# ntampellini/TSCoDe

Measured on AMD Instinct MI355X. Metric: conformers/sec, 100k x 50-atom prune_conformers pipeline (embed -> clash mask -> RMSD prune), higher is better.
Workload: dtype f64

## Files before the change

tscode_amd/csrc/local_pass.hpp:

```cpp
#pragma once
#include "rmsd.hpp"
#include "sieve.hpp"

namespace tsc {

constexpr int LP_MAX_ROWS = 2048;
constexpr int LP_WAVES = 4;
constexpr int LP_THREADS = LP_WAVES * 64;
constexpr int LP_TI = 16;
#ifndef TSC_LP_TPB
#define TSC_LP_TPB 4
#endif
constexpr int LP_TILES_PER_BLOCK = TSC_LP_TPB;
constexpr int LP_QCAP = LP_TI * 64 + 64;
constexpr int LP_WORDS = LP_MAX_ROWS / 64;
constexpr int LP_TICKET_GROUPS = 16;
#ifndef TSC_LP_OCC
#define TSC_LP_OCC 4
#endif
constexpr int LP_OCCUPANCY = TSC_LP_OCC;

struct LocalPassArgs {
    int h;
    int use_cache;
    int nb_regular;
    int nb_last;
    int c_lo;
    int n_reg;
    unsigned long long *exch;
    double thr, maxdev_thr, half_h_thr2, two_thr2, desc_limit;
    const unsigned *dmax_bits;
    unsigned long long *dbg;
};

struct LocalTickets {
    unsigned group[LP_TICKET_GROUPS][32];
    unsigned top;
    unsigned pad[31];
};

#ifdef TSC_DBG_STAMPS
#define LP_STAGE_IN(exact)                                \
    do {                                                  \
        if (!n_stages) TSC_STAMP(2);                      \
        n_stages += (exact) ? 65536 : 1;                  \
    } while (0)
#define LP_STAGE_OUT() TSC_STAMP(4)
#define LP_STAGE_COUNT()                                                                                                             \
    do {                                                                                                                             \
        if (a.dbg && (threadIdx.x & 63) == 0) a.dbg[size_t(blockIdx.x) * 32 + (threadIdx.x >> 6) * 8 + 6] = (unsigned long long)n_stages; \
    } while (0)
#else
#define LP_STAGE_IN(exact) do { } while (0)
#define LP_STAGE_OUT() do { } while (0)
#define LP_STAGE_COUNT() do { } while (0)
#endif

__device__ inline unsigned long long lds_extract64(const unsigned long long *bits, int start) {
    const int w = start >> 6, sh = start & 63;
    const unsigned long long lo = bits[w] >> sh;
    const unsigned long long hi = sh ? (bits[w + 1] << (64 - sh)) : 0ull;
    return lo | hi;
}

// ... 5 lines not shown
    unsigned long long my_sb = 0ull;
    for (int j = cv.first; j < cv.count; ++j) {
        const ViewPass vp = cv.pass[j];
        bool ok = false;
        if (removed) {
            const int c = int(((unsigned long long)unsigned(a) * vp.magic) >> vp.shift);
            if (c * vp.cs == a && c < vp.k) ok = b < ((c == vp.k - 1) ? cv.n : vp.cs * (c + 1));
        }
        unsigned long long left = __ballot(ok);
        if (!left) continue;
        unsigned long long *v = cv.views + int64_t(j) * cv.stride;
        if (ok) atomicOr(&v[b >> 6], 1ull << (b & 63));
        for (bool primary = true; left; primary = false) {
            const int leader = __ffsll((long long)left) - 1;
            const int word = __shfl(b >> 16, leader);
            const bool same = ok && (b >> 16) == word;
            unsigned long long sb = same ? 1ull << ((b >> 10) & 63) : 0ull;
            for (int off = 32; off > 0; off >>= 1) sb |= __shfl_xor(sb, off);
            if (primary) {
                if (lane == j - cv.first) my_word = int64_t(j) * cv.stride + cv.bit_words + word, my_sb = sb;
            } else if (lane == leader) {
                unsigned long long *ds = v + cv.bit_words + word;
                if ((__hip_atomic_load(ds, __ATOMIC_RELAXED, __HIP_MEMORY_SCOPE_AGENT) & sb) != sb) atomicOr(ds, sb);
            }
            left &= ~__ballot(same);
        }
    }
    if (my_sb) {
        unsigned long long *ds = cv.views + my_word;
        if ((__hip_atomic_load(ds, __ATOMIC_RELAXED, __HIP_MEMORY_SCOPE_AGENT) & my_sb) != my_sb) atomicOr(ds, my_sb);
    }
}

inline __global__ __launch_bounds__(LP_THREADS, LP_OCCUPANCY) void k_pass_chunks(PassGeom g, LocalPassArgs a, PruneState *__restrict__ st, uint8_t *__restrict__ mask,
                                                             unsigned long long *__restrict__ bits, int bit_words,
                                                             const unsigned long long *__restrict__ dbit, const double *__restrict__ heavy,
                                                             const double *__restrict__ Gall, const float *__restrict__ D,
                                                             CacheViews cv, PassCounters *__restrict__ cnt, int32_t *__restrict__ bsum, int block_items,
                                                             StepCtx sc, StepArgs next, LocalTickets *__restrict__ tickets, DeriveArgs dv) {
    __shared__ unsigned long long s_mb[LP_WORDS + 2], s_db[LP_WORDS + 2];
    __shared__ unsigned short s_wpre[LP_WORDS + 2];
    __shared__ unsigned short s_act[LP_MAX_ROWS], s_cend[LP_MAX_ROWS];
    __shared__ int s_best[LP_MAX_ROWS];
    __shared__ unsigned short s_queue[LP_WAVES][LP_QCAP], s_exq[LP_WAVES][128];
    __shared__ __attribute__((aligned(16))) float s_rowdesc[LP_WAVES][LP_TI * DW];
    __shared__ double s_jacobi[LP_WAVES][32];
    __shared__ unsigned long long s_stat[8];
    __shared__ int s_A, s_anydb, s_last, s_open[2];
    static_assert(DW == 16 && LP_TI * DW == 256, "row staging: 4 rows x 16 components per 64 lanes");

    const int tid = threadIdx.x, lane = tid & 63;
    const int wid = __builtin_amdgcn_readfirstlane(tid >> 6);
    TSC_STAMP(0);
    int c, j, nb;
    {
        const int reg_blocks = a.n_reg * a.nb_regular;
        if (int(blockIdx.x) < reg_blocks) {
            c = int(blockIdx.x) / a.nb_regular, j = int(blockIdx.x) - c * a.nb_regular, nb = a.nb_regular;
            c += a.c_lo;
        } else {
            c = g.k - 1, j = int(blockIdx.x) - reg_blocks, nb = a.nb_last;
        }
    }
    const int first = c * g.cs;
    const int L = ((c == g.k - 1) ? g.n : first + g.cs) - first;
    const int nw = (L + 63) >> 6;
// ... 54 lines not shown
        }
        __syncthreads();
        const int A = __builtin_amdgcn_readfirstlane(s_A);
        auto rank_of = [&](int t) { return int(s_wpre[t >> 6]) + __popcll(s_mb[t >> 6] & ((t & 63) ? (~0ull >> (64 - (t & 63))) : 0ull)); };
        for (int t = tid; t < L; t += LP_THREADS)
            if ((s_mb[t >> 6] >> (t & 63)) & 1ull) s_act[rank_of(t)] = (unsigned short)t;
        __syncthreads();
        const int n_tiles = (A + LP_TI - 1) / LP_TI;
        const int my_tiles = n_tiles > j ? (n_tiles - j + nb - 1) / nb : 0;
        for (int idx = tid; idx < my_tiles * LP_TI; idx += LP_THREADS) {
            const int r = (j + (idx / LP_TI) * nb) * LP_TI + (idx % LP_TI);
            if (r >= A) continue;
            const int t = s_act[r];
            int found = L;
            if (s_anydb) {
                const int len = L - t - 1;
                for (int d0 = 1; d0 <= len; d0 += 64) {
                    unsigned long long w = lds_extract64(s_mb, t + d0) & lds_extract64(s_db, d0);
                    const int rem = len - d0 + 1;
                    if (rem < 64) w &= (1ull << rem) - 1ull;
                    if (w) {
                        found = t + d0 + __ffsll((long long)w) - 1;
                        break;
                    }
                }
            }
            s_cend[r] = (unsigned short)(found >= L ? A : rank_of(found));
            s_best[r] = INT_MAX;
        }
        __syncthreads();
        TSC_STAMP(1);

        const int h3 = a.h * 3;
        const float limit32 = screen_limit32(__uint_as_float(dmax_raw), a.desc_limit);
        auto place_in = [](unsigned long long m) __attribute__((always_inline)) {
            return int(__builtin_amdgcn_mbcnt_hi(unsigned(m >> 32), __builtin_amdgcn_mbcnt_lo(unsigned(m), 0u)));
        };
        unsigned short *queue = s_queue[wid], *exq = s_exq[wid];
        float *rowdesc = s_rowdesc[wid];
        double *jac = s_jacobi[wid];
        int tile_no = 0;
        for (int rt = j; rt < n_tiles; rt += nb, ++tile_no) {
            if ((tile_no % LP_WAVES) != wid) continue;
            const int r0 = rt * LP_TI;
            const int nrows = min(LP_TI, A - r0);
            const int my_cend = lane < nrows ? int(s_cend[r0 + lane]) : 0;
            const bool live0 = lane < nrows && my_cend > r0 + lane + 1;
            unsigned alive = unsigned(__builtin_amdgcn_ballot_w64(live0));
            if (!alive) continue;
            int cmax = live0 ? my_cend : 0;
#pragma unroll
            for (int off = 32; off > 0; off >>= 1) cmax = max(cmax, __shfl_xor(cmax, off));
            cmax = __builtin_amdgcn_readfirstlane(cmax);
            float row_part[4];
#pragma unroll
            for (int q = 0; q < 4; ++q) {
                const int rr = min(r0 + 4 * q + (lane >> 4), A - 1);
                row_part[q] = D[int64_t(first + s_act[rr]) * DW + (lane & 15)];
            }
            int qn = 0, qe = 0;

            auto note_similar = [&](bool sim, int t, int col) __attribute__((always_inline)) {
                if (sim) atomicMin(&s_best[r0 + t], col);
                unsigned long long sm = __builtin_amdgcn_ballot_w64(sim);
                while (sm) {
                    const int l = __ffsll((long long)sm) - 1;
                    sm &= sm - 1;
                    alive &= ~(1u << __builtin_amdgcn_readlane(t, l));
                }
            };
            auto exact_stage = [&](int base, int cnt) __attribute__((always_inline)) {
                LP_STAGE_IN(true);
                int lpp = 64;
                while (lpp > 1 && 64 / lpp < cnt) lpp >>= 1;
                const int grp = lane / lpp, sub = lane - grp * lpp;
                bool sim = false, degenerate = false;
                int t = 0, col = 0;
                unsigned ent = 0;
                if (grp < cnt) {
                    ent = exq[base + grp];
                    t = int(ent >> 12), col = int(ent & 0xfffu);
                    const int i = first + s_act[r0 + t], jj = first + s_act[col];
                    const double *pp = heavy + int64_t(i) * h3, *pq = heavy + int64_t(jj) * h3;
                    const double Gi = Gall[i], Gj = Gall[jj];
                    double H[9], e[4];
                    pair_H(pp, pq, a.h, sub, lpp, H);
                    if (rotation_quaternion_fast(H, Gi, Gj, e)) {
                        const unsigned ent2 = reinterpret_cast<const volatile unsigned short *>(exq)[base + grp];
                        t = int(ent2 >> 12), col = int(ent2 & 0xfffu);
                        const int i2 = first + s_act[r0 + t], j2 = first + s_act[col];
                        double rm, md;
// ... 38 lines not shown
                int t = 0, col = 0;
                if (grp < cnt) {
                    e = queue[base + grp];
                    t = int(e >> 12), col = int(e & 0xfffu);
                    const int i = first + s_act[r0 + t], jj = first + s_act[col];
                    const double half_sum = 0.5 * (Gall[i] + Gall[jj]);
                    double H[9];
                    pair_H(heavy + int64_t(i) * h3, heavy + int64_t(jj) * h3, a.h, sub, lpp, H);
                    const int verdict = pair_verdict(H, half_sum, a.half_h_thr2, a.two_thr2, a.h);
                    cand = sub == 0 && verdict == PAIR_UNDECIDED;
                    sim = sub == 0 && verdict == PAIR_SIMILAR;
                }
                note_similar(sim, t, col);
                const unsigned long long m = __builtin_amdgcn_ballot_w64(cand);
                if (m) {
                    if (cand) exq[qe + place_in(m)] = (unsigned short)e;
                    qe += __popcll(m);
                }
                n_eval = __builtin_amdgcn_readfirstlane(n_eval + cnt);
                n_exact = __builtin_amdgcn_readfirstlane(n_exact + __popcll(m));
                __builtin_amdgcn_wave_barrier();
                LP_STAGE_OUT();
            };

            auto load_cols = [&](int c0, f32x2 (&dst)[KD]) __attribute__((always_inline)) {
                const f32x4 *src = reinterpret_cast<const f32x4 *>(D + int64_t(first + s_act[min(c0 + lane, A - 1)]) * DW);
#pragma unroll
                for (int k = 0; k < KD / 2; ++k) {
                    const f32x4 v = src[k];
                    dst[2 * k] = f32x2{v.x, v.y};
                    dst[2 * k + 1] = f32x2{v.z, v.w};
                }
            };
            f32x2 dq[KD], dq_next[KD];
            int c0 = (r0 + 1) & ~63;
            load_cols(c0, dq_next);
#pragma unroll
            for (int q = 0; q < 4; ++q) rowdesc[64 * q + lane] = row_part[q];
            __builtin_amdgcn_wave_barrier();
            for (bool screening = true;;) {
                if (screening) {
                    const int col = c0 + lane;
#pragma unroll
                    for (int k = 0; k < KD; ++k) dq[k] = dq_next[k];
                    if (c0 + 64 < cmax) load_cols(c0 + 64, dq_next);
                    const bool here = lane < nrows && ((alive >> lane) & 1u) && my_cend > c0 && r0 + lane < c0 + 63;
                    unsigned rows = unsigned(__builtin_amdgcn_ballot_w64(here));
                    my_screened += here ? max(0, min(my_cend, c0 + 64) - max(r0 + lane + 1, c0)) : 0;
                    while (rows) {
                        const int t = __ffs(rows) - 1;
                        rows &= rows - 1;
                        const int r = r0 + t;
                        const int ce = __builtin_amdgcn_readlane(my_cend, t);
                        const f32x2 *dr = reinterpret_cast<const f32x2 *>(rowdesc + t * DW);
                        f32x2 s2 = {0.0f, 0.0f};
#pragma unroll
                        for (int k = 0; k < KD; ++k) {
                            const f32x2 d = dr[k] - dq[k];
                            s2 = __builtin_elementwise_fma(d, d, s2);
                        }
                        const bool pass = col > r && col < ce && !(fmaxf(s2.x, s2.y) > limit32);
                        const unsigned long long m = __builtin_amdgcn_ballot_w64(pass);
                        if (m) {
                            if (pass) queue[qn + place_in(m)] = (unsigned short)((unsigned(t) << 12) | unsigned(col));
                            qn += __popcll(m);
                        }
                    }
                    c0 += 64;
                    __builtin_amdgcn_wave_barrier();
                }
                auto pending = [&]() __attribute__((always_inline)) { return qe >= 64 || qn >= 64 || (!screening && (qn | qe) != 0); };
                if (pending()) {
                    do {
                        if (qe >= 64 || qn == 0) {
                            const int cnt = min(qe, 64);
                            exact_stage(qe - cnt, cnt);
                            qe -= cnt;
                        } else {
                            const int cnt = min(qn, 64);
                            sign_stage(qn - cnt, cnt);
                            qn -= cnt;
                        }
                    } while (pending());
                    if (!screening) break;
                    load_cols(c0, dq_next);
                } else if (!screening) {
                    break;
                }
                screening = c0 < cmax && alive;
            }
        }
        for (int off = 8; off > 0; off >>= 1) my_screened += __shfl_xor(my_screened, off);
        const unsigned long long n_screened = (unsigned long long)my_screened;
        TSC_STAMP(3);
        __syncthreads();

        unsigned long long n_evaluated = 0, n_removed = 0;
        for (int rt = j; rt < n_tiles; rt += nb) {
            const int r = rt * LP_TI + lane;
            if (((rt - j) / nb) % LP_WAVES != wid) continue;
            bool removed = false;
            int my_block = -1, delta = 0;
            unsigned long long ev = 0;
            if (lane < LP_TI && r < A) {
                const int b = s_best[r];
                if (b != INT_MAX) {
                    const int t_r = s_act[r], t_b = s_act[b];
                    if (a.exch) {
                        atomicOr(&a.exch[(first + t_r) >> 6], 1ull << ((first + t_r) & 63));
                    } else {
                        mask[first + t_r] = 0;
                        atomicAnd(&mbit_next[(first + t_r) >> 6], ~(1ull << ((first + t_r) & 63)));
                        my_block = (first + t_r) / block_items;
                    }
                    delta = t_b - t_r;
                    removed = true;
                    ev = (unsigned long long)(b - r);
                } else {
                    ev = (unsigned long long)(int(s_cend[r]) - r - 1);
                }
            }
// ... 51 lines not shown
```

tscode_amd/csrc/pairs_sorted.hip:

```cpp
#include "prune_host.hpp"

int launch_rmsd_sieve_sorted(bool f32, hipStream_t st, dim3 grid, hipEvent_t e0, hipEvent_t e1, const double *heavy, const int32_t *act, const double *Gall,
                             const int32_t *cend, int32_t *best, PassCounters *counters, const PruneState *state, const SieveArgs &a, const CullArgs &ca,
                             int my_tiles, int n_seg) {
    if (f32) hipExtLaunchKernelGGL(k_rmsd_sieve_sorted<true>, grid, dim3(256), 0, st, e0, e1, 0, heavy, act, Gall, cend, best, counters, state, a, ca, my_tiles, n_seg);
    else hipExtLaunchKernelGGL(k_rmsd_sieve_sorted<false>, grid, dim3(256), 0, st, e0, e1, 0, heavy, act, Gall, cend, best, counters, state, a, ca, my_tiles, n_seg);
    TSC_HIP(hipGetLastError());
    return 0;
}

int launch_pass_chunks(hipStream_t st, unsigned blocks, hipEvent_t e0, hipEvent_t e1, const PassGeom &g, const LocalPassArgs &a, PruneState *state, uint8_t *mask,
                       unsigned long long *bits, int bit_words, const unsigned long long *view, const double *heavy, const double *Gall, const float *Dall,
                       const CacheViews &cv, PassCounters *counters, int32_t *bsum, int block_items, const StepCtx &sc, const StepArgs &sa, LocalTickets *tickets,
                       const DeriveArgs &dv) {
    hipExtLaunchKernelGGL(k_pass_chunks, dim3(blocks), dim3(LP_THREADS), 0, st, e0, e1, 0, g, a, state, mask, bits, bit_words, view, heavy, Gall, Dall, cv, counters,
                          bsum, block_items, sc, sa, tickets, dv);
    TSC_HIP(hipGetLastError());
    return 0;
}
```

tscode_amd/csrc/prune.hip:

```cpp
#include "call.hpp"
#include "prune_host.hpp"


extern "C" __attribute__((visibility("default"))) int tsc_rmsd_pairs_dev(tsc_ctx *c, const double *heavy, int64_t n_structs, int h, const int32_t *pairs, int64_t n_pairs,
                                  double *rmsd, double *maxdev) {
    TSC_API_GUARD_BEGIN
    TSC_REQUIRE(c && heavy && pairs && rmsd && maxdev, "tsc_rmsd_pairs_dev: null argument");
    TSC_REQUIRE(n_structs >= 0 && h > 0 && n_pairs >= 0, "bad sizes");
    if (n_pairs == 0) return 0;
    DeviceGuard guard(c->device);
    hipLaunchKernelGGL(k_rmsd_pairs, dim3(grid_for(n_pairs, 256)), dim3(256), 0, c->stream, heavy, h, pairs, n_pairs, rmsd, maxdev);
    TSC_HIP(hipGetLastError());
    return 0;
    TSC_API_GUARD_END
}

extern "C" __attribute__((visibility("default"))) int tsc_rmsd_pairs(tsc_ctx *c, const double *heavy, int64_t n_structs, int h, const int32_t *pairs, int64_t n_pairs,
                              double *rmsd, double *maxdev) {
    TSC_API_GUARD_BEGIN
    TSC_REQUIRE(c && heavy && pairs && rmsd && maxdev, "tsc_rmsd_pairs: null argument");
    TSC_REQUIRE(n_structs >= 0 && h > 0 && n_pairs >= 0, "bad sizes");
    for (int64_t k = 0; k < 2 * n_pairs; ++k)
        TSC_REQUIRE(pairs[k] >= 0 && pairs[k] < n_structs, "pairs[%lld] = %d out of range", (long long)k, pairs[k]);
    if (n_pairs == 0) return 0;
// ... 189 lines not shown
        p->mask = mask_buffer;
    else if (!rc)
        rc = palloc(p, size_t(n), &p->mask);
    if (!rc) rc = palloc(p, size_t(n), &p->act);
    if (!rc) rc = palloc(p, size_t(n), &p->cend);
    if (!rc) rc = palloc(p, size_t(n), &p->best);
    if (!rc) rc = palloc(p, size_t(p->n_blocks) + 1, &p->bsum);
    if (!rc) rc = palloc(p, size_t(p->n_blocks) + 1, &p->boff);
    if (!rc) rc = palloc(p, size_t(n) / 16 + 8, &p->tile_cmax);
    if (!rc) rc = palloc(p, size_t(n) / 16 + 8, &p->tile_done);
    if (!rc) rc = palloc(p, 2 * p->bit_words, &p->bits);
    p->dsum_words = p->bit_words / 1024 + 4;
    p->n_views = 0;
    for (int slot = 0; slot < TSC_MAX_PASSES; ++slot) p->view_of_slot[slot] = (pass_can_run(n, slot) && mode == 0) ? p->n_views++ : -1;
    if (!rc) rc = palloc(p, std::max<size_t>(1, size_t(p->n_views) * (p->bit_words + p->dsum_words)), &p->views);
    if (!rc) rc = palloc(p, TSC_MAX_PASSES, &p->view_pass);
    if (!rc) rc = palloc(p, TSC_MAX_PASSES, &p->counters_all);
    if (!rc) rc = palloc(p, TSC_MAX_PASSES, &p->state_all);
    p->counters = p->counters_all, p->state = p->state_all;
    if (!rc) rc = palloc(p, TSC_MAX_PASSES, &p->records);
    const bool own_desc = !(ext && ext->D);
    if (!rc && p->algo == ALGO_SIEVE) {
        if (own_desc) {
            rc = palloc(p, size_t(n) * DW, &p->Dall);
            if (!rc) rc = palloc(p, size_t(n), &p->Gall);
            if (!rc) rc = palloc(p, 4, &p->dmax_bits);
        } else {
            p->Dall = ext->D, p->Gall = ext->G, p->dmax_bits = ext->dmax_bits;
        }
        if (!rc) rc = palloc(p, size_t(n) * DW, &p->Dc);
        p->mm64 = c->opt.sieve_mm == 2 || (c->opt.sieve_mm == 1 && n >= c->opt.mm_min_n);
        const bool want_mm = p->mm64 || c->opt.sieve_mm16 != 0;
        if (!rc && want_mm) rc = palloc(p, size_t(n) * MM_REC_HALVES, &p->Dh);
        if (!rc && want_heavy32(c->opt, double(n) * h * 24.0)) {
            if (ext && ext->heavy32) {
                p->heavy32 = ext->heavy32;
            } else {
                rc = palloc(p, size_t(n) * heavy32_pitch(h), &p->heavy32);
                if (!rc) hipLaunchKernelGGL(k_heavy32, dim3(unsigned(std::min<int64_t>(ceil_div<int64_t>(n * heavy32_pitch(h), 256), 65536))), dim3(256), 0, c->stream,
                                            heavy_dev, n, h, p->heavy32);
            }
        }
    }
    if (!rc) rc = palloc(p, 1, &p->tickets);
    if (!rc && p->algo == ALGO_TILE) {
        const size_t hp3 = size_t(p->hp) * 3;
        rc = palloc(p, size_t(p->npad) * hp3, &p->Xr);
        if (!rc) rc = palloc(p, size_t(p->npad) * hp3, &p->Xc);
        if (!rc) rc = palloc(p, size_t(p->npad), &p->G);
    }
    if (!rc) {
        hipStream_t st = c->stream;
        int first_slot = -1;
        for (int slot = 0; slot < TSC_MAX_PASSES && first_slot < 0; ++slot)
            if (pass_can_run(n, slot)) first_slot = slot;
        p->opened_slot = first_slot;
        InitArgs ia;
        memset(&ia, 0, sizeof(ia));
        ia.n = n, ia.mask = p->mask, ia.bits = p->bits, ia.bit_words = int(p->bit_words);
        ia.views = p->views, ia.view_words = int64_t(p->n_views) * int64_t(p->bit_words + p->dsum_words), ia.view_pass = p->view_pass, ia.n_views = p->n_views;
        for (int slot = 0; slot < TSC_MAX_PASSES; ++slot)
            if (p->view_of_slot[slot] >= 0) ia.sched[p->view_of_slot[slot]] = view_pass(int(n), int(KS[slot]));
        ia.st = p->state_all, ia.rec = p->records, ia.n_rec = TSC_MAX_PASSES, ia.cnt = p->counters_all;
        ia.bsum = p->bsum, ia.boff = p->boff, ia.n_blocks = p->n_blocks, ia.block_items = SCAN_TILE;
        ia.dmax_bits = own_desc ? p->dmax_bits : nullptr;
        ia.zero_words = reinterpret_cast<unsigned *>(p->tickets), ia.n_zero_words = int64_t(sizeof(*p->tickets) / sizeof(unsigned));
        ia.act = p->act, ia.first_slot = first_slot, ia.first_k = first_slot >= 0 ? (long long)KS[first_slot] : 0ll, ia.first_algo = p->algo;
        ia.tile_done = p->tile_done, ia.n_tile_done = n / 16 + 8;
        hipLaunchKernelGGL(k_init_run, dim3(grid_for(n / 8 + 1, 256, 512)), dim3(256), 0, st, ia);
        hipError_t e = hipGetLastError();
        if (e == hipSuccess && p->Xc) e = hipMemsetAsync(p->Xc, 0, size_t(p->npad) * p->hp * 3 * sizeof(double), st);
        if (e == hipSuccess && p->Xr) e = hipMemsetAsync(p->Xr, 0, size_t(p->npad) * p->hp * 3 * sizeof(double), st);
        if (e == hipSuccess && p->G) e = hipMemsetAsync(p->G, 0, size_t(p->npad) * sizeof(double), st);
        if (e != hipSuccess) rc = fail(TSC_ERR_HIP, "prune state setup failed: %s", hipGetErrorString(e));
    }
    if (!rc && p->Dall && own_desc) rc = build_descriptors(p, basis);
    if (rc) {
        tsc_prune_destroy(p);
        return rc;
    }
    *out = p;
    return 0;
}


extern "C" __attribute__((visibility("default"))) int tsc_prune_create(tsc_ctx *c, const double *heavy_dev, int64_t n, int h, double rmsd_thr, int mode, tsc_prune **out) {
    TSC_API_GUARD_BEGIN
    TSC_REQUIRE(c != nullptr, "tsc_prune_create: null argument");
    if (c->xd_valid && c->xd_h == h && c->xd_heavy == heavy_dev && n <= c->xd_cap && c->opt.prune_algo != ALGO_TILE) {
        ExternalDescriptors ext;
        ext.D = c->xd_D, ext.G = c->xd_G, ext.dmax_bits = c->xd_dmax;
        ext.heavy32 = c->xd_h32_valid ? c->xd_heavy32 : nullptr;
        c->xd_valid = false;
        TSC_TRY(prune_create_impl(c, heavy_dev, n, h, rmsd_thr, mode, nullptr, out, nullptr, &ext));
        std::lock_guard<std::mutex> lock(c->runs_mutex);
        (*out)->borrows_xd = true;
        ++c->xd_borrowers;
        return 0;
    }
    c->xd_valid = false;
    const double *basis = pending_basis(c, h);
    if (basis) {
        DeviceGuard guard(c->device);
        TSC_HIP(hipStreamWaitEvent(c->stream, c->ev_join, 0));
    }
    c->eb_valid = false;
    return prune_create_impl(c, heavy_dev, n, h, rmsd_thr, mode, nullptr, out, basis);
    TSC_API_GUARD_END
}
// ... 103 lines not shown
        fa.tile_done = p->tile_done, fa.tickets = p->cur_range ? &p->tickets->pass : nullptr, fa.n_tiles = unsigned(w.n_tiles);
        fa.sc = step_ctx(p, p->cur_range);
        int nxt = -1;
        fa.next = next_step_args(p, &nxt);
        if (!p->cur_range) p->last_local = false;
    }
    const bool trim = c->opt.sieve_cpl == 2 && c->opt.sieve_trim;
    if (form.mm16) {
        TSC_TRY(launch_rmsd_sieve_mm16(p->cur_fused, a.heavy32 != nullptr, w.mm16_waves, st, w.grid, ev.e0, ev.e1, p->heavy, (const int32_t *)p->act,
                                       (const double *)p->Gall, (const _Float16 *)p->Dh, (const int32_t *)p->cend, p->best, p->counters,
                                       (const PruneState *)p->state, a, fa));
        return 0;
    }
    if (form.mm) {
        TSC_TRY(launch_rmsd_sieve_mm(p->cur_fused, a.heavy32 != nullptr, st, w.grid, ev.e0, ev.e1, p->heavy, (const int32_t *)p->act, (const double *)p->Gall,
                                     (const float *)p->Dc, (const _Float16 *)p->Dh, (const int32_t *)p->cend, p->best, p->counters, (const PruneState *)p->state, a,
                                     fa));
        return 0;
    }
    TSC_TRY((p->cur_fused ? launch_rmsd_sieve_fused : launch_rmsd_sieve_plain)(
        c->opt.sieve_cpl, trim, trim && a.heavy32 != nullptr, st, w.grid, ev.e0, ev.e1, p->heavy, (const int32_t *)p->act, (const double *)p->Gall, (const float *)p->Dc,
        (const int32_t *)p->cend, p->best, p->counters, (const PruneState *)p->state, a, fa));
    TSC_HIP(hipGetLastError());
    return 0;
}

static int local_pass(tsc_prune *p, const PassGeom &g, const PassRows &r, bool range) {
    const LocalPlan l = plan_local(p->n, p->cur_k, r);
    LocalPassArgs a;
    a.h = p->h, a.use_cache = (p->mode == 0);
    a.nb_regular = l.nb_regular, a.nb_last = l.nb_last;
    a.c_lo = int(r.c_lo), a.n_reg = l.n_reg;
    a.exch = range ? p->exch : nullptr;
    a.dbg = nullptr;
#ifdef TSC_DBG_STAMPS
    if (p->ctx->opt.dbg_stamp_k == p->cur_k) TSC_TRY(stamp_buffer(p->ctx, int64_t(l.blocks) * 4, &a.dbg));
#endif
    put_screen_thresholds(p, a);
    int nxt = -1;
    const StepArgs sa = next_step_args(p, &nxt);
    const PairEvents ev = pair_events(p, 2);
    TSC_TRY(launch_pass_chunks(p->ctx->stream, unsigned(l.blocks), ev.e0, ev.e1, g, a, p->state, p->mask, p->bits, int(p->bit_words), view_of_open_pass(p), p->heavy,
                               (const double *)p->Gall, (const float *)p->Dall, later_views(p), p->counters, p->bsum, SCAN_TILE, step_ctx(p, range), sa,
                               range ? &p->tickets->local : nullptr, derive_args(p)));
    if (!range) p->last_local = true;
    return 0;
}

static int open_rows(tsc_prune *p, const PassGeom &g, const PassShape &s, bool range) {
    tsc_ctx *c = p->ctx;
    hipStream_t st = c->stream;
    const OpenPlan o = plan_open_rows(s.rows_ub);
    OpenArgs oa;
    oa.use_cache = (p->mode == 0), oa.fused = (s.fused && range) ? 1 : 0, oa.lds_cap = std::min(c->opt.open_lds_blocks, OPEN_LDS_BLOCKS);
    oa.view = view_of_open_pass(p), oa.bits = p->bits, oa.bit_words = int(p->bit_words);
    oa.boff = p->boff, oa.n_blocks = p->n_blocks, oa.block_items = SCAN_TILE;
    oa.n_tiles = o.n_tiles, oa.tickets = &p->tickets->pass;
    oa.dv = derive_args(p), oa.bsum = p->bsum, oa.boff_out = p->boff;
    oa.rank_of = s.culled ? p->rank_of : nullptr;
    oa.Dh = p->Dh, oa.dmax_bits = p->dmax_bits;
    oa.dbg = nullptr;
#ifdef TSC_DBG_STAMPS
    if (c->opt.dbg_stamp_k == -p->cur_k) TSC_TRY(stamp_buffer(c, int64_t(o.stamp_blocks) * 4, &oa.dbg));
#endif
    int nxt = -1;
    const StepArgs sa = s.fused ? next_step_args(p, &nxt) : StepArgs{-1, -1, 0ll, 0, -1};
    static_assert(SCAN_TILE == 64 * SCAN_BLOCK_WORDS && DW == DESC_WORDS, "k_open_rows");
    hipLaunchKernelGGL(k_open_rows, dim3(o.blocks), dim3(256), 0, st, g, oa, step_ctx(p, range), sa, p->act, p->cend, p->best, p->tile_cmax, (const float *)p->Dall,
                       s.need_dc ? p->Dc : nullptr);
    if (p->algo == ALGO_TILE) {
        const int hp3 = p->hp * 3;
        size_t lds = size_t(64) * (hp3 + 1) * sizeof(double);
        hipLaunchKernelGGL(k_compact_coords, dim3(ceil_div(s.rows_ub, 64)), dim3(256), lds, st, p->heavy, p->h, hp3, p->act, (const PruneState *)p->state, p->Xr,
                           p->Xc, p->npad, p->G);
    }
// ... 561 lines not shown
```

tscode_amd/csrc/prune_host.hpp:

```cpp
#pragma once

#include "pass_plan.hpp"
#include "scan.hpp"


static const double KS[TSC_MAX_PASSES] = {5e5, 2e5, 1e5, 5e4, 2e4, 1e4, 5000, 2000, 1000, 500, 200, 100, 50, 20, 10, 5, 2, 1};

static_assert(MAX_SLOTS == TSC_MAX_PASSES, "one cache view per schedule slot");

static inline bool pass_can_run(int64_t n, int slot) {
    const int64_t k = int64_t(KS[slot]);
    return k == 1 || 20 * k < n;
}

struct tsc_prune {
    tsc_ctx *ctx = nullptr;
    const double *heavy = nullptr;
    int64_t n = 0, npad = 0;
    int h = 0, hp = 0;
    double thr = 0;
    int mode = 0;
    int algo = ALGO_SIEVE;
    uint8_t *mask = nullptr;
    int32_t *act = nullptr, *cend = nullptr, *best = nullptr;
    int32_t *bsum = nullptr, *boff = nullptr, *tile_cmax = nullptr, *tile_done = nullptr;
    int n_blocks = 0;
    unsigned long long *bits = nullptr;
    unsigned long long *views = nullptr;
    ViewPass *view_pass = nullptr;
    int view_of_slot[TSC_MAX_PASSES];
    int n_views = 0;
    size_t bit_words = 0, dsum_words = 0;
    bool cur_fused = false;
    double *Xr = nullptr, *Xc = nullptr, *G = nullptr;
    float *Dall = nullptr;
    float *Dc = nullptr;
    bool mm64 = false;
    _Float16 *Dh = nullptr;
    double *Gall = nullptr;
    struct Tickets {
        PassTickets pass;
        LocalTickets local;
    } *tickets = nullptr;
    bool cur_local = false;
    int32_t *morton_order = nullptr, *rank_of = nullptr, *crank = nullptr, *cbase = nullptr, *cfill = nullptr, *blk_cnt = nullptr;
    float *Ds = nullptr, *cbox = nullptr, *rbox = nullptr;
    int32_t *cstruct = nullptr;
    _Float16 *Dhs = nullptr;
    float *heavy32 = nullptr;
    bool morton_sorted = false;
    int part_rank = 0, part_world = 1, part_min_chunks = 0;
    unsigned long long *exch = nullptr;
    bool cur_range = false;
    int range_ready_slot = -1;
    bool views_split = false;
    uint8_t *export_mask_host = nullptr;
    unsigned *dmax_bits = nullptr;
    PassCounters *counters_all = nullptr;
    PruneState *state_all = nullptr;
    PassCounters *counters = nullptr;
    PruneState *state = nullptr;
    PassRecord *records = nullptr;
    std::vector<void *> blocks;
    int next_ks = 0;
    int cur_slot = -1;
    int last_slot = -1;
    int opened_slot = -1;
    bool derive_prev = false;
    int derive_slot = -1;
    bool last_local = false, derive_local = false;
    int64_t cur_k = 0;
// ... 65 lines not shown
static inline const unsigned long long *view_of_open_pass(const tsc_prune *p) {
    return p->mode == 0 ? p->views + size_t(p->view_of_slot[p->cur_slot]) * (p->bit_words + p->dsum_words) : p->views;
}

static inline ApplyArgs apply_args(const tsc_prune *p) {
    ApplyArgs a;
    a.g = PassGeom{int(p->n), int(p->cur_k), int(p->n / p->cur_k)};
    a.act = p->act, a.cend = p->cend, a.best = p->best, a.mask = p->mask, a.bits = p->bits, a.bit_words = int(p->bit_words);
    a.bsum = p->bsum, a.block_items = SCAN_TILE, a.cv = later_views(p);
    a.exch = p->cur_range ? p->exch : nullptr;
    return a;
}

int launch_rmsd_tile(int hp, hipStream_t st, dim3 grid, hipEvent_t e0, hipEvent_t e1, const double *Xr, const double *Xc, const double *G, const int32_t *cend,
                     int32_t *best, PassCounters *counters, const PruneState *state, const TileArgs &a);
int launch_rmsd_sieve_fused(int cpl, bool trim, bool f32, hipStream_t st, dim3 grid, hipEvent_t e0, hipEvent_t e1, const double *heavy, const int32_t *act,
                            const double *Gall, const float *Dc, const int32_t *cend, int32_t *best, PassCounters *counters, const PruneState *state,
                            const SieveArgs &a, const FusedApply &fa);
int launch_rmsd_sieve_plain(int cpl, bool trim, bool f32, hipStream_t st, dim3 grid, hipEvent_t e0, hipEvent_t e1, const double *heavy, const int32_t *act,
                            const double *Gall, const float *Dc, const int32_t *cend, int32_t *best, PassCounters *counters, const PruneState *state,
                            const SieveArgs &a, const FusedApply &fa);
int launch_rmsd_sieve_mm(bool fused, bool f32, hipStream_t st, dim3 grid, hipEvent_t e0, hipEvent_t e1, const double *heavy, const int32_t *act, const double *Gall,
                         const float *Dc, const _Float16 *Dh, const int32_t *cend, int32_t *best, PassCounters *counters, const PruneState *state, const SieveArgs &a,
                         const FusedApply &fa);
int launch_rmsd_sieve_sorted(bool f32, hipStream_t st, dim3 grid, hipEvent_t e0, hipEvent_t e1, const double *heavy, const int32_t *act, const double *Gall,
                             const int32_t *cend, int32_t *best, PassCounters *counters, const PruneState *state, const SieveArgs &a, const CullArgs &ca,
                             int my_tiles, int n_seg);
int launch_rmsd_sieve_mm16(bool fused, bool f32, int waves, hipStream_t st, dim3 grid, hipEvent_t e0, hipEvent_t e1, const double *heavy, const int32_t *act, const double *Gall,
                           const _Float16 *Dh, const int32_t *cend, int32_t *best, PassCounters *counters, const PruneState *state,
                           const SieveArgs &a, const FusedApply &fa);
int launch_rmsd_sieve_sorted_mm(bool f32, hipStream_t st, dim3 grid, hipEvent_t e0, hipEvent_t e1, const double *heavy, const int32_t *act, const double *Gall,
                                const int32_t *cend, int32_t *best, PassCounters *counters, const PruneState *state, const SieveArgs &a, const CullArgs &ca,
                                const CullMmArgs &cm, int n_groups, int n_seg);
int launch_pass_chunks(hipStream_t st, unsigned blocks, hipEvent_t e0, hipEvent_t e1, const PassGeom &g, const LocalPassArgs &a, PruneState *state, uint8_t *mask,
                       unsigned long long *bits, int bit_words, const unsigned long long *view, const double *heavy, const double *Gall, const float *Dall,
                       const CacheViews &cv, PassCounters *counters, int32_t *bsum, int block_items, const StepCtx &sc, const StepArgs &sa, LocalTickets *tickets,
                       const DeriveArgs &dv);
```

tscode_amd/csrc/rmsd.hpp:

```cpp
#pragma once
#include "common.hpp"
#include "mm_record.hpp"
#include "scan.hpp"

namespace tsc {


__device__ inline void top_eigvec4(double A[4][4], double q[4]) {
    double V[4][4];
#pragma unroll
    for (int i = 0; i < 4; ++i)
#pragma unroll
        for (int j = 0; j < 4; ++j) V[i][j] = (i == j) ? 1.0 : 0.0;
    for (int sweep = 0; sweep < 16; ++sweep) {
        double off = 0.0, dia = 0.0;
#pragma unroll
        for (int i = 0; i < 4; ++i) {
            dia += A[i][i] * A[i][i];
#pragma unroll
            for (int j = i + 1; j < 4; ++j) off += A[i][j] * A[i][j];
        }
        if (!(off > 1e-30 * dia)) break;
#pragma unroll
        for (int p = 0; p < 3; ++p) {
// ... 301 lines not shown
                unsigned long long *ds = v + cv.bit_words + word;
                if ((__hip_atomic_load(ds, __ATOMIC_RELAXED, __HIP_MEMORY_SCOPE_AGENT) & sb) != sb) atomicOr(ds, sb);
            }
            left &= ~__ballot(same);
        }
    }
}

struct InitArgs {
    int64_t n;
    uint8_t *mask;
    unsigned long long *bits;
    int bit_words;
    unsigned long long *views;
    int64_t view_words;
    ViewPass *view_pass;
    int n_views;
    ViewPass sched[MAX_SLOTS];
    PruneState *st;
    PassRecord *rec;
    int n_rec;
    PassCounters *cnt;
    int32_t *bsum, *boff;
    int n_blocks, block_items;
    unsigned *dmax_bits;
    unsigned *zero_words;
    int64_t n_zero_words;
    int32_t *tile_done;
    int64_t n_tile_done;
    int32_t *act;
    int first_slot;
    long long first_k;
    int first_algo;
};
inline __global__ __launch_bounds__(256) void k_init_run(InitArgs a) {
    const int64_t n = a.n;
    const int64_t tid = int64_t(blockIdx.x) * blockDim.x + threadIdx.x, stride = int64_t(gridDim.x) * blockDim.x;
    unsigned long long *m8 = reinterpret_cast<unsigned long long *>(a.mask);
    for (int64_t e = tid; e < n / 8; e += stride) m8[e] = 0x0101010101010101ull;
    for (int64_t e = (n / 8) * 8 + tid; e < n; e += stride) a.mask[e] = 1;
    for (int64_t e = tid; e < n; e += stride) a.act[e] = int32_t(e);
    for (int64_t e = tid; e < a.bit_words; e += stride) {
        const int64_t lo = e * 64;
        const unsigned long long w = lo + 64 <= n ? ~0ull : (lo >= n ? 0ull : ((1ull << (n - lo)) - 1ull));
        a.bits[e] = w, a.bits[a.bit_words + e] = w;
    }
    for (int64_t e = tid; e < a.view_words; e += stride) a.views[e] = 0;
    unsigned long long *c = &a.cnt->w[0][0];
    for (int64_t e = tid; e < int64_t(MAX_SLOTS) * CNT_BUCKETS * CNT_WORDS; e += stride) c[e] = 0;
    for (int64_t e = tid; e < a.n_zero_words; e += stride) a.zero_words[e] = 0;
    for (int64_t e = tid; e < a.n_tile_done; e += stride) a.tile_done[e] = 0;
    char *r = reinterpret_cast<char *>(a.rec);
    for (int64_t e = tid; e < int64_t(a.n_rec) * int64_t(sizeof(PassRecord)); e += stride)
        if (int(e / int64_t(sizeof(PassRecord))) != a.first_slot) r[e] = 0;
    for (int64_t e = tid; e <= a.n_blocks; e += stride) {
        const int64_t lo = e * a.block_items;
        if (e < a.n_blocks) a.bsum[e] = int32_t(lo >= n ? 0 : (n - lo < a.block_items ? n - lo : a.block_items));
        a.boff[e] = int32_t(lo >= n ? n : lo);
    }
    if (tid < a.n_views) a.view_pass[tid] = a.sched[tid];
    if (tid == 0) {
        if (a.dmax_bits) *a.dmax_bits = 0;
        for (int s = 0; s < MAX_SLOTS; ++s) {
            PruneState *ss = a.st + s;
            ss->n_active = int(n), ss->pass_on = 0, ss->A = int(n), ss->ticket = 0, ss->bitsel = 0, ss->row_lo = 0, ss->cull_on = 0;
        }
        PruneState *st = a.st + (a.first_slot >= 0 ? a.first_slot : 0);
        if (a.first_slot >= 0) {
            const int on = (a.first_k == 1 || 20 * a.first_k < (long long)n) ? 1 : 0;
            PassRecord &fr = a.rec[a.first_slot];
            fr.k = a.first_k, fr.n_before = fr.n_after = (long long)n, fr.on = on, fr.algo = a.first_algo;
            fr.formed = fr.exact = fr.screened = fr.evaluated = fr.removed = 0;
            st->pass_on = on;
        }
// ... 957 lines not shown
```

Measured before the change: 152.0 million.

## Screen chunk-local pass pairs with f16 MFMA descriptor records

Adds an MFMA-based screening path to the chunk-local pass kernel, templated on MM. It builds f16 descriptor records, either in the init kernel or in a separate kernel, and computes 16x16 similarity blocks with mfma_f32_16x16x16f16. Threshold hits are extracted via sign bits and pushed into the exact-stage queue. This replaces the scalar f32 per-lane descriptor screen. It costs extra memory for the records plus a record-building pass, and relies on the conservativeness of the f16 screening bound.

```diff
diff --git a/tscode_amd/csrc/local_pass.hpp b/tscode_amd/csrc/local_pass.hpp
--- a/tscode_amd/csrc/local_pass.hpp
+++ b/tscode_amd/csrc/local_pass.hpp
@@ -1,6 +1,7 @@
 #pragma once
 #include "rmsd.hpp"
 #include "sieve.hpp"
+#include "mm.hpp"
 
 namespace tsc {
 
@@ -30,6 +31,7 @@
     unsigned long long *exch;
     double thr, maxdev_thr, half_h_thr2, two_thr2, desc_limit;
     const unsigned *dmax_bits;
+    const _Float16 *rec;
     unsigned long long *dbg;
 };
 
@@ -101,6 +103,9 @@
     }
 }
 
+constexpr int LP_MM_BLOCKS = 64 / MM_STEP;
+
+template <bool MM>
 inline __global__ __launch_bounds__(LP_THREADS, LP_OCCUPANCY) void k_pass_chunks(PassGeom g, LocalPassArgs a, PruneState *__restrict__ st, uint8_t *__restrict__ mask,
                                                              unsigned long long *__restrict__ bits, int bit_words,
                                                              const unsigned long long *__restrict__ dbit, const double *__restrict__ heavy,
@@ -221,7 +226,9 @@
         TSC_STAMP(1);
 
         const int h3 = a.h * 3;
-        const float limit32 = screen_limit32(__uint_as_float(dmax_raw), a.desc_limit);
+        [[maybe_unused]] const float limit32 = MM ? 0.0f : screen_limit32(__uint_as_float(dmax_raw), a.desc_limit);
+        [[maybe_unused]] const float limit_mm = MM ? __uint_as_float(__builtin_amdgcn_readfirstlane(__float_as_uint(screen_limit_mm(dmax_raw, a.desc_limit)))) : 0.0f;
+        [[maybe_unused]] const int g4 = lane >> 4, rc = lane & 15;
         auto place_in = [](unsigned long long m) __attribute__((always_inline)) {
             return int(__builtin_amdgcn_mbcnt_hi(unsigned(m >> 32), __builtin_amdgcn_mbcnt_lo(unsigned(m), 0u)));
         };
@@ -241,11 +248,18 @@
 #pragma unroll
             for (int off = 32; off > 0; off >>= 1) cmax = max(cmax, __shfl_xor(cmax, off));
             cmax = __builtin_amdgcn_readfirstlane(cmax);
-            float row_part[4];
-#pragma unroll
-            for (int q = 0; q < 4; ++q) {
-                const int rr = min(r0 + 4 * q + (lane >> 4), A - 1);
-                row_part[q] = D[int64_t(first + s_act[rr]) * DW + (lane & 15)];
+            [[maybe_unused]] float row_part[4];
+            [[maybe_unused]] f16x4 Ar[NFAM];
+            if constexpr (MM) {
+                const _Float16 *rr = a.rec + int64_t(first + s_act[min(r0 + rc, A - 1)]) * MM_REC_HALVES;
+#pragma unroll
+                for (int fam = 0; fam < NFAM; ++fam) Ar[fam] = mm_load_A(rr, fam, g4);
+            } else {
+#pragma unroll
+                for (int q = 0; q < 4; ++q) {
+                    const int rr = min(r0 + 4 * q + (lane >> 4), A - 1);
+                    row_part[q] = D[int64_t(first + s_act[rr]) * DW + (lane & 15)];
+                }
             }
             int qn = 0, qe = 0;
 
@@ -350,14 +364,73 @@
                     dst[2 * k + 1] = f32x2{v.z, v.w};
                 }
             };
-            f32x2 dq[KD], dq_next[KD];
+            auto load_recs = [&](int c0, f16x4 (&dst)[LP_MM_BLOCKS][NFAM]) __attribute__((always_inline)) {
+#pragma unroll
+                for (int b = 0; b < LP_MM_BLOCKS; ++b)
+                    mm_load_B2(a.rec + int64_t(first + s_act[min(c0 + MM_STEP * b + rc, A - 1)]) * MM_REC_HALVES, g4, dst[b]);
+            };
+            static_assert(NFAM == 2 && LP_TI * DW == 64 * 4, "a lane's two operands are the 16 bytes at its place in the row area");
+            auto put_rows = [&]() __attribute__((always_inline)) {
+                const f32x2 lo = __builtin_bit_cast(f32x2, Ar[0]), hi = __builtin_bit_cast(f32x2, Ar[1]);
+                *reinterpret_cast<f32x4 *>(rowdesc + 4 * lane) = f32x4{lo.x, lo.y, hi.x, hi.y};
+            };
+            auto get_rows = [&]() __attribute__((always_inline)) {
+                const f32x4 v = *reinterpret_cast<const f32x4 *>(rowdesc + 4 * lane);
+                const f32x2 lo = {v.x, v.y}, hi = {v.z, v.w};
+                Ar[0] = __builtin_bit_cast(f16x4, lo), Ar[1] = __builtin_bit_cast(f16x4, hi);
+                if (g4 == 2 && !((alive >> rc) & 1u)) Ar[0][0] = _Float16(__builtin_inff());
+            };
+            [[maybe_unused]] f32x2 dq[KD], dq_next[KD];
+            [[maybe_unused]] f16x4 Bq[LP_MM_BLOCKS][NFAM];
             int c0 = (r0 + 1) & ~63;
-            load_cols(c0, dq_next);
-#pragma unroll
-            for (int q = 0; q < 4; ++q) rowdesc[64 * q + lane] = row_part[q];
+            if constexpr (MM) {
+                put_rows();
+            } else {
+                load_cols(c0, dq_next);
+#pragma unroll
+                for (int q = 0; q < 4; ++q) rowdesc[64 * q + lane] = row_part[q];
+            }
             __builtin_amdgcn_wave_barrier();
             for (bool screening = true;;) {
-                if (screening) {
+                if constexpr (MM) {
+                    if (screening) {
+                        load_recs(c0, Bq);
+                        const bool here = lane < nrows && ((alive >> lane) & 1u) && my_cend > c0 && r0 + lane < c0 + 63;
+                        my_screened += here ? max(0, min(my_cend, c0 + 64) - max(r0 + lane + 1, c0)) : 0;
+                        get_rows();
+                        unsigned m0 = 0, m1 = 0;
+#pragma unroll
+                        for (int b = 0; b < LP_MM_BLOCKS; ++b) {
+                            const f32x4 z = {-limit_mm, -limit_mm, -limit_mm, -limit_mm};
+                            const f32x4 s0 = __builtin_amdgcn_mfma_f32_16x16x16f16(Ar[0], Bq[b][0], z, 0, 0, 0);
+                            const f32x4 s1 = __builtin_amdgcn_mfma_f32_16x16x16f16(Ar[1], Bq[b][1], z, 0, 0, 0);
+#pragma unroll
+                            for (int i = 0; i < 4; ++i) {
+                                m0 = __builtin_amdgcn_alignbit(m0, __float_as_uint(s0[i]), 31);
+                                m1 = __builtin_amdgcn_alignbit(m1, __float_as_uint(s1[i]), 31);
+                            }
+                        }
+                        static_assert(4 * LP_MM_BLOCKS == 16, "16 values per lane and family: moved to the top half for the count of leading zeros");
+                        unsigned hits = (m0 & m1) << 16;
+                        while (__builtin_amdgcn_ballot_w64(hits != 0u)) {
+                            bool keep = false;
+                            unsigned ent = 0;
+                            if (hits) {
+                                const int jv = __builtin_clz(hits);
+                                hits &= ~(0x80000000u >> jv);
+                                const int row = 4 * g4 + (jv & 3), col = c0 + MM_STEP * (jv >> 2) + rc;
+                                keep = col > r0 + row && ((alive >> row) & 1u) && col < int(s_cend[r0 + row]);
+                                ent = (unsigned(row) << 12) | unsigned(col);
+                            }
+                            const unsigned long long km = __builtin_amdgcn_ballot_w64(keep);
+                            if (keep) queue[qn + place_in(km)] = (unsigned short)ent;
+                            qn += __popcll(km);
+                        }
+                        c0 += 64;
+                        alive &= ~unsigned(__builtin_amdgcn_ballot_w64(lane < nrows && ((alive >> lane) & 1u) && my_cend <= c0));
+                        __builtin_amdgcn_wave_barrier();
+                    }
+                } else if (screening) {
                     const int col = c0 + lane;
 #pragma unroll
                     for (int k = 0; k < KD; ++k) dq[k] = dq_next[k];
@@ -399,12 +472,14 @@
                             sign_stage(qn - cnt, cnt);
                             qn -= cnt;
                         }
+                        if constexpr (MM) alive = unsigned(__builtin_amdgcn_readfirstlane(int(alive)));
                     } while (pending());
                     if (!screening) break;
-                    load_cols(c0, dq_next);
+                    if constexpr (!MM) load_cols(c0, dq_next);
                 } else if (!screening) {
                     break;
                 }
+                if constexpr (MM) alive = unsigned(__builtin_amdgcn_readfirstlane(int(alive)));
                 screening = c0 < cmax && alive;
             }
         }
diff --git a/tscode_amd/csrc/pairs_sorted.hip b/tscode_amd/csrc/pairs_sorted.hip
--- a/tscode_amd/csrc/pairs_sorted.hip
+++ b/tscode_amd/csrc/pairs_sorted.hip
@@ -9,12 +9,14 @@
     return 0;
 }
 
-int launch_pass_chunks(hipStream_t st, unsigned blocks, hipEvent_t e0, hipEvent_t e1, const PassGeom &g, const LocalPassArgs &a, PruneState *state, uint8_t *mask,
+int launch_pass_chunks(bool mm, hipStream_t st, unsigned blocks, hipEvent_t e0, hipEvent_t e1, const PassGeom &g, const LocalPassArgs &a, PruneState *state, uint8_t *mask,
                        unsigned long long *bits, int bit_words, const unsigned long long *view, const double *heavy, const double *Gall, const float *Dall,
                        const CacheViews &cv, PassCounters *counters, int32_t *bsum, int block_items, const StepCtx &sc, const StepArgs &sa, LocalTickets *tickets,
                        const DeriveArgs &dv) {
-    hipExtLaunchKernelGGL(k_pass_chunks, dim3(blocks), dim3(LP_THREADS), 0, st, e0, e1, 0, g, a, state, mask, bits, bit_words, view, heavy, Gall, Dall, cv, counters,
-                          bsum, block_items, sc, sa, tickets, dv);
+    if (mm) hipExtLaunchKernelGGL(k_pass_chunks<true>, dim3(blocks), dim3(LP_THREADS), 0, st, e0, e1, 0, g, a, state, mask, bits, bit_words, view, heavy, Gall, Dall, cv,
+                                  counters, bsum, block_items, sc, sa, tickets, dv);
+    else hipExtLaunchKernelGGL(k_pass_chunks<false>, dim3(blocks), dim3(LP_THREADS), 0, st, e0, e1, 0, g, a, state, mask, bits, bit_words, view, heavy, Gall, Dall, cv,
+                               counters, bsum, block_items, sc, sa, tickets, dv);
     TSC_HIP(hipGetLastError());
     return 0;
 }
diff --git a/tscode_amd/csrc/prune.hip b/tscode_amd/csrc/prune.hip
--- a/tscode_amd/csrc/prune.hip
+++ b/tscode_amd/csrc/prune.hip
@@ -245,6 +245,10 @@
         p->mm64 = c->opt.sieve_mm == 2 || (c->opt.sieve_mm == 1 && n >= c->opt.mm_min_n);
         const bool want_mm = p->mm64 || c->opt.sieve_mm16 != 0;
         if (!rc && want_mm) rc = palloc(p, size_t(n) * MM_REC_HALVES, &p->Dh);
+        bool local_possible = false;
+        for (int slot = 0; slot < TSC_MAX_PASSES; ++slot)
+            local_possible = local_possible || (pass_can_run(n, slot) && n / int64_t(KS[slot]) <= std::min(LP_MAX_ROWS, c->opt.local_max_chunk));
+        if (!rc && c->opt.sieve_mm16 != 0 && c->opt.local_pass != 0 && local_possible) rc = palloc(p, size_t(n) * MM_REC_HALVES, &p->Drec);
         if (!rc && want_heavy32(c->opt, double(n) * h * 24.0)) {
             if (ext && ext->heavy32) {
                 p->heavy32 = ext->heavy32;
@@ -280,7 +284,9 @@
         ia.zero_words = reinterpret_cast<unsigned *>(p->tickets), ia.n_zero_words = int64_t(sizeof(*p->tickets) / sizeof(unsigned));
         ia.act = p->act, ia.first_slot = first_slot, ia.first_k = first_slot >= 0 ? (long long)KS[first_slot] : 0ll, ia.first_algo = p->algo;
         ia.tile_done = p->tile_done, ia.n_tile_done = n / 16 + 8;
-        hipLaunchKernelGGL(k_init_run, dim3(grid_for(n / 8 + 1, 256, 512)), dim3(256), 0, st, ia);
+        const bool rec_here = p->Drec && !own_desc;
+        if (rec_here) ia.Dall = p->Dall, ia.rec_dmax_bits = p->dmax_bits, ia.mm_rec = p->Drec;
+        hipLaunchKernelGGL(k_init_run, dim3(grid_for(n / (rec_here ? 2 : 8) + 1, 256, 512)), dim3(256), 0, st, ia);
         hipError_t e = hipGetLastError();
         if (e == hipSuccess && p->Xc) e = hipMemsetAsync(p->Xc, 0, size_t(p->npad) * p->hp * 3 * sizeof(double), st);
         if (e == hipSuccess && p->Xr) e = hipMemsetAsync(p->Xr, 0, size_t(p->npad) * p->hp * 3 * sizeof(double), st);
@@ -288,6 +294,10 @@
         if (e != hipSuccess) rc = fail(TSC_ERR_HIP, "prune state setup failed: %s", hipGetErrorString(e));
     }
     if (!rc && p->Dall && own_desc) rc = build_descriptors(p, basis);
+    if (!rc && p->Drec && own_desc) {
+        hipLaunchKernelGGL(k_mm_records, dim3(grid_for(n, 256, 1024)), dim3(256), 0, c->stream, (const float *)p->Dall, n, (const unsigned *)p->dmax_bits, p->Drec);
+        if (hipGetLastError() != hipSuccess) rc = fail(TSC_ERR_HIP, "the records of the chunk-local pass could not be written");
+    }
     if (rc) {
         tsc_prune_destroy(p);
         return rc;
@@ -457,6 +467,7 @@
     a.nb_regular = l.nb_regular, a.nb_last = l.nb_last;
     a.c_lo = int(r.c_lo), a.n_reg = l.n_reg;
     a.exch = range ? p->exch : nullptr;
+    a.rec = p->ctx->opt.sieve_mm16 != 0 ? p->Drec : nullptr;
     a.dbg = nullptr;
 #ifdef TSC_DBG_STAMPS
     if (p->ctx->opt.dbg_stamp_k == p->cur_k) TSC_TRY(stamp_buffer(p->ctx, int64_t(l.blocks) * 4, &a.dbg));
@@ -465,7 +476,7 @@
     int nxt = -1;
     const StepArgs sa = next_step_args(p, &nxt);
     const PairEvents ev = pair_events(p, 2);
-    TSC_TRY(launch_pass_chunks(p->ctx->stream, unsigned(l.blocks), ev.e0, ev.e1, g, a, p->state, p->mask, p->bits, int(p->bit_words), view_of_open_pass(p), p->heavy,
+    TSC_TRY(launch_pass_chunks(a.rec != nullptr, p->ctx->stream, unsigned(l.blocks), ev.e0, ev.e1, g, a, p->state, p->mask, p->bits, int(p->bit_words), view_of_open_pass(p), p->heavy,
                                (const double *)p->Gall, (const float *)p->Dall, later_views(p), p->counters, p->bsum, SCAN_TILE, step_ctx(p, range), sa,
                                range ? &p->tickets->local : nullptr, derive_args(p)));
     if (!range) p->last_local = true;
diff --git a/tscode_amd/csrc/prune_host.hpp b/tscode_amd/csrc/prune_host.hpp
--- a/tscode_amd/csrc/prune_host.hpp
+++ b/tscode_amd/csrc/prune_host.hpp
@@ -37,6 +37,7 @@
     float *Dc = nullptr;
     bool mm64 = false;
     _Float16 *Dh = nullptr;
+    _Float16 *Drec = nullptr;
     double *Gall = nullptr;
     struct Tickets {
         PassTickets pass;
@@ -168,7 +169,7 @@
 int launch_rmsd_sieve_sorted_mm(bool f32, hipStream_t st, dim3 grid, hipEvent_t e0, hipEvent_t e1, const double *heavy, const int32_t *act, const double *Gall,
                                 const int32_t *cend, int32_t *best, PassCounters *counters, const PruneState *state, const SieveArgs &a, const CullArgs &ca,
                                 const CullMmArgs &cm, int n_groups, int n_seg);
-int launch_pass_chunks(hipStream_t st, unsigned blocks, hipEvent_t e0, hipEvent_t e1, const PassGeom &g, const LocalPassArgs &a, PruneState *state, uint8_t *mask,
+int launch_pass_chunks(bool mm, hipStream_t st, unsigned blocks, hipEvent_t e0, hipEvent_t e1, const PassGeom &g, const LocalPassArgs &a, PruneState *state, uint8_t *mask,
                        unsigned long long *bits, int bit_words, const unsigned long long *view, const double *heavy, const double *Gall, const float *Dall,
                        const CacheViews &cv, PassCounters *counters, int32_t *bsum, int block_items, const StepCtx &sc, const StepArgs &sa, LocalTickets *tickets,
                        const DeriveArgs &dv);
diff --git a/tscode_amd/csrc/rmsd.hpp b/tscode_amd/csrc/rmsd.hpp
--- a/tscode_amd/csrc/rmsd.hpp
+++ b/tscode_amd/csrc/rmsd.hpp
@@ -357,6 +357,9 @@
     int first_slot;
     long long first_k;
     int first_algo;
+    const float *Dall;
+    const unsigned *rec_dmax_bits;
+    _Float16 *mm_rec;
 };
 inline __global__ __launch_bounds__(256) void k_init_run(InitArgs a) {
     const int64_t n = a.n;
@@ -365,6 +368,18 @@
     for (int64_t e = tid; e < n / 8; e += stride) m8[e] = 0x0101010101010101ull;
     for (int64_t e = (n / 8) * 8 + tid; e < n; e += stride) a.mask[e] = 1;
     for (int64_t e = tid; e < n; e += stride) a.act[e] = int32_t(e);
+    if (a.mm_rec) {
+        const float sigma = mm_scale(*a.rec_dmax_bits);
+        for (int64_t e = tid; e < n; e += stride) {
+            float d[2 * MM_KD];
+#pragma unroll
+            for (int q = 0; q < MM_KD / 2; ++q) {
+                const float4 v = *reinterpret_cast<const float4 *>(a.Dall + e * (2 * MM_KD) + 4 * q);
+                d[4 * q] = v.x, d[4 * q + 1] = v.y, d[4 * q + 2] = v.z, d[4 * q + 3] = v.w;
+            }
+            mm_write_record(d, sigma, a.mm_rec + e * MM_REC_HALVES);
+        }
+    }
     for (int64_t e = tid; e < a.bit_words; e += stride) {
         const int64_t lo = e * 64;
         const unsigned long long w = lo + 64 <= n ? ~0ull : (lo >= n ? 0ull : ((1ull << (n - lo)) - 1ull));
```

After: 155.8 million, median of 6. 1.02x the previous value.
